# laurentsenta/testground

Hardware: AMD Instinct MI355X
Metric: simulated packets/sec (whole node) at 10k & 1M peers; % of HBM roofline (higher is better)
Workload: dtype u32/u64 integer

## Files before the change

include/tgsim.h:

```cpp
#ifndef TGSIM_H
#define TGSIM_H

#include <stddef.h>
#include <stdint.h>

#ifdef __cplusplus
extern "C" {
#endif

#define TGSIM_ABI_VERSION 2u

#define TGSIM_EXTERNAL 0xFFFFFFFFu

enum tgsim_filter { TGSIM_ACCEPT = 0, TGSIM_REJECT = 1, TGSIM_DROP = 2 };

enum tgsim_policy { TGSIM_POLICY_UNSET = 0, TGSIM_ALLOW_ALL = 1, TGSIM_DENY_ALL = 2 };

enum tgsim_verdict {
    TGSIM_V_SCHEDULED = 0,
    TGSIM_V_DISCONNECTED = 1,
    TGSIM_V_NO_ROUTE = 2,
    TGSIM_V_BLACKHOLE = 3,
    TGSIM_V_PROHIBIT = 4,
    TGSIM_V_LOSS = 5,
// ... 341 lines not shown
uint64_t tgsim_bridge_now_tick(void* bridge);
int tgsim_udp_front_create(void* bridge, uint16_t port, void** out_front);
int tgsim_udp_front_port(void* front);
int tgsim_udp_front_register(void* front, uint32_t peer, uint32_t ipv4, uint16_t port);
int tgsim_udp_front_bind_peer(void* front, uint32_t peer, uint32_t ipv4, uint16_t port);
int64_t tgsim_udp_front_pump(void* front);
void tgsim_udp_front_destroy(void* front);

double tgsim_sim_kernel_ms(void* engine, uint64_t* n_launches, int reset);
double tgsim_delivery_kernel_ms(void* engine, uint64_t* n_windows, int reset);
void* tgsim_stream(void* engine);
int64_t tgsim_debug_stamps(void* engine, uint64_t* out, size_t cap);
int64_t tgsim_debug_carry_bytes(void* engine);
int64_t tgsim_debug_bucket_records(void* engine);
int64_t tgsim_debug_fused_windows(void* engine);
int64_t tgsim_debug_sparse_windows(void* engine);
int64_t tgsim_debug_exec_faults(void);

#ifdef __cplusplus
}
#endif

#endif
```

testground_amd/abi.py:

```python
from __future__ import annotations

import ctypes as C

import numpy as np

ABI_VERSION = 2
EXTERNAL = 0xFFFFFFFF

V_SCHEDULED, V_DISCONNECTED, V_NO_ROUTE, V_BLACKHOLE, V_PROHIBIT, V_LOSS, V_QUEUE_FULL, V_EXTERNAL = range(8)
V_NONE = 15
VERDICT_NAMES = ["scheduled", "disconnected", "no_route", "blackhole", "prohibit", "loss",
                 "queue_full", "external"]

FLAG_DUP = 0x1
FLAG_CORRUPT = 0x2

OPT_DISCARD_DELIVERIES = 0x2
OPT_METRICS = 0x4
OPT_K8S = 0x8
SYNC_STATES = 65536
METRICS_SRC, METRICS_DST, METRICS_HIST = 0, 1, 2
METRICS_SRC_WORDS, METRICS_DST_WORDS, METRICS_BINS = 12, 2, 64
METRICS_SRC_COLUMNS = ["offered", "offered_bytes"] + [f"verdict_{i}" for i in range(8)] + ["served", "served_bytes"]

# ... 203 lines not shown
assert C.sizeof(FlowSummary) == 120
assert C.sizeof(FlowCC) == 16 and FLOW_CC_ROW_DTYPE.itemsize == 32 and C.sizeof(FlowCCSummary) == 64
assert C.sizeof(FlowRto) == 16 and FLOW_RTO_ROW_DTYPE.itemsize == 32 and C.sizeof(FlowRtoSummary) == 64
assert C.sizeof(FlowFb) == 16 and FLOW_FB_ROW_DTYPE.itemsize == 32 and C.sizeof(FlowFbSummary) == 96
assert C.sizeof(CommInfo) == 72 and C.sizeof(Gossip) == 24 and C.sizeof(Opts) == 56 and C.sizeof(Shape) == 56 and C.sizeof(Config) == 104

EXPORTS = [
    "tgsim_create", "tgsim_destroy", "tgsim_last_error", "tgsim_abi_version", "tgsim_configure",
    "tgsim_configure_batch", "tgsim_link_generation",
    "tgsim_submit", "tgsim_gen_storm", "tgsim_step", "tgsim_step_sim", "tgsim_deliver",
    "tgsim_deliver_async", "tgsim_wait_event", "tgsim_sync", "tgsim_step_sim_launch", "tgsim_step_sim_finish",
    "tgsim_step_sim_counts", "tgsim_delivery_event", "tgsim_step_sim_launch_slotted", "tgsim_step_sim_release",
    "tgsim_deliver_slotted_async", "tgsim_step_sim_launch_slotted_n", "tgsim_deliver_slotted_n_async",
    "tgsim_sim_capacity", "tgsim_drain", "tgsim_pending_deliveries", "tgsim_verdicts", "tgsim_stats",
    "tgsim_signal", "tgsim_signal_async", "tgsim_barrier_poll", "tgsim_sync_counters", "tgsim_sim_kernel_ms", "tgsim_delivery_kernel_ms", "tgsim_stream", "tgsim_debug_stamps",
    "tgsim_debug_fused_windows", "tgsim_debug_sparse_windows", "tgsim_debug_carry_bytes", "tgsim_debug_bucket_records", "tgsim_debug_exec_faults", "tgsim_step_n",
    "tgsim_gossip_init", "tgsim_gen_gossip", "tgsim_gossip_reached", "tgsim_gossip_spread",
    "tgsim_gossip_times", "tgsim_metrics",
    "tgsim_ping_init", "tgsim_gen_ping", "tgsim_ping_report", "tgsim_ping_pairs",
    "tgsim_flow_init", "tgsim_gen_flow", "tgsim_flow_report", "tgsim_flow_rows",
    "tgsim_flow_init_cc", "tgsim_flow_cc_rows", "tgsim_flow_cc_report",
    "tgsim_flow_init_rto", "tgsim_flow_rto_rows", "tgsim_flow_rto_report",
    "tgsim_flow_init_fb", "tgsim_flow_fb_rows", "tgsim_flow_fb_report",
    "tgsim_groups_init", "tgsim_group_matrix",
    "tgsim_comm_id", "tgsim_comm_init", "tgsim_comm_step", "tgsim_comm_launch", "tgsim_comm_finish", "tgsim_comm_run", "tgsim_comm_barrier", "tgsim_comm_info",
    "tgsim_bridge_create", "tgsim_bridge_destroy", "tgsim_bridge_send", "tgsim_bridge_step",
    "tgsim_bridge_recv", "tgsim_bridge_pending", "tgsim_bridge_in_flight", "tgsim_bridge_now_tick",
    "tgsim_bridge_link_removed",
    "tgsim_udp_front_create", "tgsim_udp_front_port", "tgsim_udp_front_register", "tgsim_udp_front_bind_peer",
    "tgsim_udp_front_pump", "tgsim_udp_front_destroy",
]
# ... 37 lines not shown
    f("sync", C.c_int, vp)
    f("sim_capacity", C.c_int64, vp)
    f("drain", C.c_int64, vp, C.c_void_p, C.c_size_t)
    f("pending_deliveries", C.c_int64, vp)
    f("verdicts", C.c_int64, vp, C.c_void_p, C.c_size_t)
    f("stats", C.c_int, vp, C.POINTER(Stats))
    f("signal", C.c_int64, vp, C.c_uint32, C.c_uint32)
    f("barrier_poll", C.c_int, vp, C.c_uint32, C.c_uint64)
    f("signal_async", C.c_int, vp, C.c_uint32, C.c_uint32)
    f("sync_counters", C.c_int, vp, C.POINTER(vp), C.POINTER(C.c_uint32), vp)
    f("sim_kernel_ms", C.c_double, vp, C.POINTER(C.c_uint64), C.c_int)
    f("delivery_kernel_ms", C.c_double, vp, C.POINTER(C.c_uint64), C.c_int)
    f("stream", vp, vp)
    f("debug_stamps", C.c_int64, vp, C.c_void_p, C.c_size_t)
    f("debug_fused_windows", C.c_int64, vp)
    f("debug_sparse_windows", C.c_int64, vp)
    f("debug_exec_faults", C.c_int64)
    f("debug_carry_bytes", C.c_int64, vp)
    f("debug_bucket_records", C.c_int64, vp)
    f("abi_version", C.c_uint32)
    f("gossip_init", C.c_int, vp, C.POINTER(Gossip))
    f("gen_gossip", C.c_int, vp, C.c_uint32)
    f("gossip_reached", C.c_int64, vp, C.c_void_p, C.c_size_t)
    f("gossip_spread", C.c_int64, vp, C.c_uint32, C.c_uint32, C.c_void_p, C.c_void_p, C.c_size_t)
    f("gossip_times", C.c_int64, vp, C.c_uint32, C.c_uint32, C.c_void_p, C.c_size_t)
    f("ping_init", C.c_int, vp, C.POINTER(Ping), C.c_void_p)
    f("gen_ping", C.c_int, vp, C.c_uint32)
    f("ping_report", C.c_int64, vp, C.POINTER(PingSummary), C.c_void_p, C.c_size_t)
    f("ping_pairs", C.c_int64, vp, C.c_uint32, C.c_uint32, C.c_void_p, C.c_size_t)
    f("flow_init", C.c_int, vp, C.POINTER(Flow), C.c_void_p, C.c_uint64)
# ... 26 lines not shown
```

testground_amd/csrc/tgsim_comm.cpp:

```cpp
#include <dlfcn.h>
#include <sched.h>
#include <errno.h>
#include <stdarg.h>
#include <stdio.h>
#include <stdlib.h>
#include <string.h>

#include <algorithm>
#include <chrono>
#include <string>
#include <vector>

#include <rccl/rccl.h>

#include "tgsim_launch.h"

using namespace tgsim;

namespace {

constexpr size_t kRec = sizeof(tgsim_delivery);
constexpr uint32_t kRoutedGridPct = 90;

struct Rccl {
// ... 453 lines not shown
  CRC(tgsim_deliver_async(e, C->in[i].p, roff[nr], C->ev_out[j]));
  CRC(tgsim_delivery_event(e, C->ev_in[i]));
  C->in_busy[i] = true;
  return 0;
}

int tgsim_comm_step(void* e, uint32_t n_ticks) {
  int rc = tgsim_comm_launch(e, n_ticks);
  return rc ? rc : tgsim_comm_finish(e);
}

int tgsim_comm_run(void* e, uint32_t n_ticks, uint32_t n_steps, uint32_t fuse, uint64_t slot_cap) {
  Comm* C = comm_of(e);
  if (!C) return e ? engine_fail(e, -EINVAL, "comm_run: no communicator (tgsim_comm_init)") : -EINVAL;
  if (C->timed_out) return -ETIMEDOUT;
  if (n_ticks == 0 || fuse == 0 || fuse > kFuseMax) return -EINVAL;
  if (C->launched) return engine_fail(e, -EBUSY, "comm_run: a launched window is not finished (tgsim_comm_finish)");
  if (engine_ping_armed(e)) return engine_fail(e, -EBUSY, "comm_run: the ping driver is armed (single engine, tgsim_step)");
  if (engine_flow_armed(e)) return engine_fail(e, -EBUSY, "comm_run: the flow driver is armed (single engine, tgsim_step)");
  if (!n_steps) return 0;
  CHIP(hipSetDevice(C->dev));
  const int nr = C->nranks;
  if (C->local) {
    CRC(tgsim_step_n(e, n_ticks, n_steps));
    C->k += n_steps;
    return 0;
  }
  if (!slot_cap) {
    uint64_t mx = 0;
    if (nr == 1) CRC(engine_route_max(e, &C->max_count));
    C->h_cnt[0] = C->max_count;
// ... 95 lines not shown
```

testground_amd/csrc/tgsim_engine.cpp:

```cpp
#include <errno.h>
#include <stdlib.h>
#include <stdarg.h>
#include <stdio.h>
#include <string.h>

#include <algorithm>
#include <array>
#include <cmath>
#include <map>
#include <numeric>
#include <string>
#include <thread>
#include <unordered_map>
#include <vector>

#include "tgsim_launch.h"

using namespace tgsim;

inline void spin_pause() {
#if defined(__x86_64__) || defined(__i386__)
  __builtin_ia32_pause();
#endif
}
// ... 322 lines not shown
  bool stamps_on = false;
  DevBuf<uint32_t> d_order;
  DevBuf<uint32_t> d_work;
  int sparse_mode = -1;
  bool rotated = false;
  bool sparse_seen = false;
  uint32_t dense_streak = 0;
  static constexpr uint32_t dense_div = 4;
  bool order_valid = false;
  struct LocalSet {
    DevBuf<tgsim_delivery> emit;
    DevBuf<uint32_t> emit_n;
  };
  LocalSet fset[2][kFuseMax];
  DevBuf<uint64_t> f_lcnt[2];
  hipEvent_t ev_fgrp[2] = {};
  uint32_t fgrp = 0;
  DevBuf<uint8_t> f_verdict[kFuseMax];
  DevBuf<uint32_t> d_done, d_ticket;
  uint32_t step_no = 0, ticket_no = 0;
  uint64_t fused_windows = 0;
  uint64_t sparse_windows = 0;
  uint32_t fused_wgs = 0;
  uint32_t routed_pct = 0;
  CommSlot comm{};
  static constexpr uint32_t prio_heavy = 512;
  int fuse_max = 8;
  DevBuf<uint64_t> d_stamps;
  uint64_t n_stamp_wg = 0;

  bool metrics_on = false;
  DevBuf<unsigned long long> d_msrc, d_mdst, d_mhist;

  bool gossip_on = false;
  bool gossip_late = false;
  tgsim_gossip gossip{};
  DevBuf<uint32_t> d_gfirst, d_gerr, d_gnbr;
  DevBuf<uint64_t> d_gfwd, d_gpend;
  DevBuf<uint64_t> d_gspread;
  DevBuf<uint32_t> d_gtimes;

  bool ping_on = false;
// ... 1241 lines not shown
  if (rc) return rc;
  HIPCHK(hipEventRecord(E->ev_dst, sq));
  rotate_emit(E);
  return 0;
}

bool fusable(Eng* E, uint32_t n_ticks, uint32_t g, bool routed = false) {
  if (g < 2 || (E->S != E->N && !routed) || !E->staged.empty() || E->gen_q.size() < g || E->metrics_on ||
      E->gossip_on || E->ping_on || E->flow_on || E->groups_on || E->sparse_mode == 1 || kSpw != 1)
    return false;
  for (uint32_t i = 0; i < g; ++i)
    if (E->gen_q[i].ticks != n_ticks || E->gen_q[i].n < 64ull * E->S) return false;
  return true;
}

struct GroupRoute {
  uint32_t n_ranks;
  const uint32_t* bounds;
  tgsim_delivery* out;
  uint64_t slot_cap;
  hipEvent_t routed;
};

int step_fused(Eng* E, uint32_t n_ticks, uint32_t g, const GroupRoute* gr = nullptr) {
  int rc = check_sim_error(E);
  if (rc) return rc;
  rc = harvest_timing(E, false);
  if (rc) return rc;
  rc = flush_config(E);
  if (rc) return rc;
// ... 9 lines not shown
    E->rotated = false;
  }
  if (E->d_done.cap < E->S) {
    HIPCHK(E->d_done.ensure(E->S));
    HIPCHK(hipMemsetAsync(E->d_done.p, 0, sizeof(uint32_t) * E->d_done.cap, E->st));
    HIPCHK(E->d_ticket.ensure(1));
    HIPCHK(hipMemsetAsync(E->d_ticket.p, 0, sizeof(uint32_t), E->st));
    E->step_no = E->ticket_no = 0;
  }
  ensure_wheel(E);
  SimArgs a = base_sim_args(E);
  const bool ordered = E->S <= kOrderMaxSources;
  a.order = ordered && E->order_valid ? E->d_order.p : nullptr;
  FusedArgs f{};
  const uint64_t nseg = static_cast<uint64_t>(g) * E->N;
  for (auto& lc : E->f_lcnt)
    if (lc.cap < static_cast<uint64_t>(kFuseMax) * E->N) {
      HIPCHK(lc.ensure(static_cast<uint64_t>(kFuseMax) * E->N));
      HIPCHK(hipMemsetAsync(lc.p, 0, sizeof(uint64_t) * lc.cap, E->st));
    }
  uint64_t rec_bound = 0, n_max = 0;
  for (uint32_t i = 0; i < g; ++i) {
    rec_bound += 2 * win[i].n + static_cast<uint64_t>(kHeapCap) * E->S;
    n_max = std::max(n_max, win[i].n);
  }
  const uint32_t n_sets = std::max(static_cast<uint32_t>(E->fuse_max), g);
  for (auto& grp : E->fset)
    for (uint32_t i = 0; i < n_sets; ++i) {
      HIPCHK(grp[i].emit.ensure(2 * n_max + static_cast<uint64_t>(kHeapCap) * E->S));
      HIPCHK(grp[i].emit_n.ensure(E->S));
    }
  HIPCHK(E->d_verdict.ensure(n_max ? n_max : 1));
  for (uint32_t i = 0; i + 1 < n_sets; ++i) HIPCHK(E->f_verdict[i].ensure(n_max ? n_max : 1));
  if (!gr) {
    const uint64_t segs = static_cast<uint64_t>(E->fuse_max) * E->N;
    const uint64_t recs = static_cast<uint64_t>(E->fuse_max) * (2 * n_max + static_cast<uint64_t>(kHeapCap) * E->S);
    HIPCHK(E->d_doff.ensure(segs + 1));
    HIPCHK(E->d_dpos.ensure(segs));
    HIPCHK(E->d_dblk.ensure((segs + 1023) / 1024 + 1));
    HIPCHK(E->d_scatter.ensure(recs));
    if (E->o.flags & TGSIM_OPT_DISCARD_DELIVERIES) HIPCHK(E->d_sorted.ensure(recs));
  }
  for (uint32_t i = 0; i < g; ++i) {
    Eng::LocalSet& ls = E->fset[p][i];
    DevBuf<uint8_t>& vb = i + 1 == g ? E->d_verdict : E->f_verdict[i];
    const uint64_t t0 = (E->now_tick + static_cast<uint64_t>(i) * n_ticks) * E->o.tick_ns;
    f.w[i] = {win[i].off.p, win[i].in.p, vb.p, ls.emit.p, ls.emit_n.p,
              gr ? nullptr : reinterpret_cast<unsigned long long*>(E->f_lcnt[p].p + static_cast<uint64_t>(i) * E->N),
              t0, t0 + n_ticks * E->o.tick_ns + E->o.lookahead_ns};
  }
  a.stamps = nullptr;
  if (E->stamps_on) {
    HIPCHK(E->d_stamps.ensure(static_cast<size_t>(g) * E->S * kStampSlots));
    a.stamps = E->d_stamps.p;
    E->n_stamp_wg = static_cast<uint64_t>(g) * E->S;
  }
  f.n_win = g;
  f.prio_n = a.order ? E->prio_heavy : 0;
  f.step_base = E->step_no;
  f.ticket_base = E->ticket_no;
  f.ticket = E->d_ticket.p;
  f.done = E->d_done.p;
  hipEvent_t ev0, ev1;
  HIPCHK(take_event(E, &ev0));
  HIPCHK(take_event(E, &ev1));
  HIPCHK(hipEventRecord(ev0, E->st));
  if (!E->fused_wgs) {
    E->fused_wgs = sim_fused_resident();
  }
  f.persistent = gr ? (E->routed_pct ? 1u : 0u) : 1u;
  const uint32_t wgs = gr && E->routed_pct ? std::max(1u, E->fused_wgs * std::min(E->routed_pct, 100u) / 100u)
                                           : E->fused_wgs;
  launch_sim_fused(a, f, wgs, E->st);
  HIPCHK(hipGetLastError());
  E->sim_calls++;
  HIPCHK(hipEventRecord(ev1, E->st));
  E->ev_pending.push_back({ev0, ev1, g});
  E->step_no += g;
  const uint32_t tickets = g * E->S;
  E->ticket_no += tickets + (f.persistent ? std::min(wgs, tickets) : 0u);
  E->fused_windows += g;
  if (ordered) {
    HIPCHK(E->d_order.ensure(E->S));
    launch_order(E->fset[p][g - 1].emit_n.p, E->S, E->d_order.p, E->st);
    HIPCHK(hipGetLastError());
    E->order_valid = true;
  }
  if (gr) {
    hipStream_t rs = E->rt_st;
    HIPCHK(hipEventRecord(E->ev_sim, E->st));
    HIPCHK(hipStreamWaitEvent(rs, E->ev_sim, 0));
    const uint64_t m = static_cast<uint64_t>(gr->n_ranks) * E->S;
    HIPCHK(E->d_rcnt.ensure(m));
    HIPCHK(E->d_rpos.ensure(m + 1));
    HIPCHK(E->d_rblk.ensure((m + 1023) / 1024 + 1));
    HIPCHK(E->d_rtot.ensure(1));
// ... 235 lines not shown
        return bail(rc);
      }
  }
  if (const char* ec = getenv("TGSIM_EMIT_COMPACT")) E->emit_compact = std::min(std::max(atoi(ec), 0), 2);
  if (const char* ds = getenv("TGSIM_DST_SLOT")) E->dst_slot = atoi(ds) != 0;
  if (const char* db = getenv("TGSIM_DST_BKT")) E->dst_bkt = atoi(db) != 0;
  E->emit_sets = E->S == E->N ? 3u : 2u;
  if (const char* es = getenv("TGSIM_EMIT_SETS")) E->emit_sets = atoi(es) == 2 ? 2u : 3u;
  if (const char* er = getenv("TGSIM_EMIT_R")) E->emit_r = static_cast<uint32_t>(std::min(std::max(1, atoi(er)), 1024));
  if (const char* ep = getenv("TGSIM_EMIT_POOL")) E->emit_pool = static_cast<uint32_t>(std::min(std::max(0, atoi(ep)), 4096));
  if (const char* ds = getenv("TGSIM_DELIVER_SLACK")) {
    E->deliver_slack = strtoull(ds, nullptr, 10);
    E->slack_forced = true;
  }
  if (const char* fz = getenv("TGSIM_FUSE")) E->fuse_max = std::max(1, std::min(atoi(fz), static_cast<int>(kFuseMax)));
  for (hipEvent_t& ev : E->ev_fgrp) {
    if ((rc = E->hip(hipEventCreateWithFlags(&ev, kEvSync), "event"))) return bail(rc);
    if ((rc = E->hip(hipEventRecord(ev, E->dst_st), "event"))) return bail(rc);
  }
  E->enabled.assign(E->N, 1);
  E->ip6_set.assign(E->N, 0);
  E->ip6.resize(E->N);
  E->k8s_init.assign(E->N, 0);
  E->gone.assign(E->N, 0);
  E->link_gen.assign(E->N, 0);
  E->ip.resize(E->N);
  for (uint32_t i = 0; i < E->N; ++i) E->ip[i] = E->o.subnet_base + 2 + i;
  E->src.resize(E->S);
  for (uint32_t s = 0; s < E->S; ++s) reset_source(E, s);
  E->patch_n = 0;
// ... 78 lines not shown
  E->d_drain.release(); E->d_gfirst.release(); E->d_gfwd.release(); E->d_gpend.release(); E->d_gnbr.release(); E->d_gerr.release(); E->d_gspread.release(); E->d_gtimes.release(); E->d_stats.release(); E->d_stamps.release(); E->d_order.release();
  E->d_msrc.release(); E->d_mdst.release(); E->d_mhist.release(); E->d_work.release(); E->d_rsend.release();
  for (auto* q : {&E->gen_q, &E->gen_free})
    for (auto& w : *q) {
      w.off.release();
      w.in.release();
    }
  for (auto* pend : {&E->ev_pending, &E->dv_pending})
    for (auto& pr : *pend) {
      (void)hipEventDestroy(pr.first);
      (void)hipEventDestroy(pr.second);
    }
  for (auto& grp : E->fset)
    for (auto& ls : grp) { ls.emit.release(); ls.emit_n.release(); }
  for (auto& v : E->f_lcnt) v.release();
  for (auto& v : E->f_verdict) v.release();
  E->d_done.release(); E->d_ticket.release();
  for (hipEvent_t ev : E->ev_fgrp)
    if (ev) (void)hipEventDestroy(ev);
  for (hipEvent_t ev : E->ev_pool) (void)hipEventDestroy(ev);
  if (E->h_err) (void)hipHostFree(E->h_err);
  if (E->h_xerr) (void)hipHostFree(E->h_xerr);
  if (E->h_work) (void)hipHostFree(E->h_work);
  flow_release(E);
  groups_release(E);
  if (E->h_ppub) (void)hipHostFree(E->h_ppub);
  if (E->ev_ping) (void)hipEventDestroy(E->ev_ping);
  if (E->ev_flow) (void)hipEventDestroy(E->ev_flow);
  if (E->ev_fb) (void)hipEventDestroy(E->ev_fb);
  if (E->h_gerr) (void)hipHostFree(E->h_gerr);
// ... 1014 lines not shown
  if (!E || n_ticks == 0 || n_ranks == 0 || n_ranks > 8 || !bounds || !d_out || slot_cap == 0) return -EINVAL;
  if (bounds[0] != 0 || bounds[n_ranks] != E->N) return E->fail(-EINVAL, "rank bounds must cover [0, n_peers)");
  if (E->route_n == Eng::kRouteSlots) return E->fail(-EBUSY, "two launched steps are not released yet");
  if (E->ping_on) return E->fail(-EBUSY, "%s: the ping driver is armed (tgsim_ping_init(engine, NULL, NULL) disarms it)", "step_sim_launch_slotted");
  if (E->flow_on) return E->fail(-EBUSY, "%s: the flow driver is armed (tgsim_flow_init(engine, NULL, NULL, 0) disarms it)", "step_sim_launch_slotted");
  HIPCHK(hipSetDevice(E->dev));
  int rc = run_sim(E, n_ticks);
  if (rc) return rc;
  return route_launch(E, n_ranks, bounds, static_cast<tgsim_delivery*>(d_out), n_ranks * (slot_cap + 1), slot_cap,
                      static_cast<hipEvent_t>(routed_event));
}

int tgsim_step_sim_launch_slotted_n(void* e, uint32_t n_ticks, uint32_t n_win, uint32_t n_ranks,
                                    const uint32_t* bounds, void* d_out, uint64_t slot_cap, void* routed_event) {
  Eng* E = as_eng(e);
  if (!E || n_ticks == 0 || n_win == 0 || n_win > kFuseMax || n_ranks == 0 || n_ranks > 8 || !bounds || !d_out ||
      slot_cap == 0)
    return -EINVAL;
  if (n_win == 1)
    return tgsim_step_sim_launch_slotted(e, n_ticks, n_ranks, bounds, d_out, slot_cap, routed_event);
  if (bounds[0] != 0 || bounds[n_ranks] != E->N) return E->fail(-EINVAL, "rank bounds must cover [0, n_peers)");
  if (E->route_n == Eng::kRouteSlots) return E->fail(-EBUSY, "two launched steps are not released yet");
  if (E->ping_on) return E->fail(-EBUSY, "%s: the ping driver is armed (tgsim_ping_init(engine, NULL, NULL) disarms it)", "step_sim_launch_slotted_n");
  if (E->flow_on) return E->fail(-EBUSY, "%s: the flow driver is armed (tgsim_flow_init(engine, NULL, NULL, 0) disarms it)", "step_sim_launch_slotted_n");
  HIPCHK(hipSetDevice(E->dev));
  if (!fusable(E, n_ticks, n_win, true))
    return E->fail(-EINVAL, "step_sim_launch_slotted_n: the next %u windows are not generated dense windows of %u ticks",
                   n_win, n_ticks);
  const GroupRoute gr{n_ranks, bounds, static_cast<tgsim_delivery*>(d_out), slot_cap, static_cast<hipEvent_t>(routed_event)};
  return step_fused(E, n_ticks, n_win, &gr);
}

int tgsim_deliver_slotted_n_async(void* e, const void* d_in, uint32_t n_ranks, uint32_t n_win, uint64_t slot_cap,
                                  void* wait_event) {
  Eng* E = as_eng(e);
  if (!E || !d_in || n_ranks == 0 || n_ranks > 8 || n_win == 0 || n_win > kFuseMax || slot_cap == 0) return -EINVAL;
  HIPCHK(hipSetDevice(E->dev));
  return deliver(E, static_cast<const tgsim_delivery*>(d_in), static_cast<uint64_t>(n_ranks) * n_win * (slot_cap + 1),
                 static_cast<hipEvent_t>(wait_event), false, slot_cap, n_win);
}

int tgsim_step_sim_release(void* e) {
  Eng* E = as_eng(e);
  if (!E) return -EINVAL;
  if (!E->route_n) return E->fail(-EINVAL, "no routed step pending");
  HIPCHK(hipSetDevice(E->dev));
  E->route_head = (E->route_head + 1) % Eng::kRouteSlots;
  E->route_n--;
  int rc = harvest_timing(E, false);
  if (rc) return rc;
  return check_sim_error(E);
// ... 76 lines not shown
  HIPCHK(E->d_bucket.ensure(cap));
  const uint32_t bounds[2] = {0, E->N};
  uint64_t count = 0;
  rc = route(E, 1, bounds, E->d_bucket.p, E->d_bucket.cap, &count);
  if (rc) return rc;
  rc = deliver(E, E->d_bucket.p, count, nullptr, true);
  if (rc) return rc;
  return finish_sim_timing(E);
}

int tgsim_step_n(void* e, uint32_t n_ticks, uint32_t n_steps) {
  Eng* E = as_eng(e);
  if (!E || n_ticks == 0) return -EINVAL;
  if (E->route_n) return E->fail(-EBUSY, "launched steps are not finished yet");
  HIPCHK(hipSetDevice(E->dev));
  while (n_steps) {
    const uint32_t g = std::min(n_steps, static_cast<uint32_t>(E->fuse_max));
    int rc;
    if (fusable(E, n_ticks, g)) {
      rc = step_fused(E, n_ticks, g);
      n_steps -= g;
    } else {
      rc = tgsim_step(e, n_ticks);
      n_steps -= 1;
    }
    if (rc) return rc;
  }
  return 0;
}

int64_t tgsim_link_generation(void* e, uint32_t peer) {
  Eng* E = as_eng(e);
  if (!E || peer >= E->N) return -EINVAL;
// ... 195 lines not shown
  return static_cast<int64_t>(n);
}

int64_t tgsim_debug_exec_faults(void) { return exec_faults(); }

int64_t tgsim_debug_sparse_windows(void* e) {
  Eng* E = as_eng(e);
  return E ? static_cast<int64_t>(E->sparse_windows) : -EINVAL;
}

int64_t tgsim_debug_fused_windows(void* e) {
  Eng* E = as_eng(e);
  return E ? static_cast<int64_t>(E->fused_windows) : -EINVAL;
}

void* tgsim_stream(void* e) {
  Eng* E = as_eng(e);
  return E ? static_cast<void*>(E->st) : nullptr;
}

int tgsim_host_compile_shape(const tgsim_shape* s, uint64_t out[13]) {
  if (!s || !out) return -EINVAL;
  const Compiled c = compile_shape(*s);
  out[0] = c.p.lat_ns; out[1] = static_cast<uint64_t>(static_cast<int64_t>(c.p.sigma));
  out[2] = static_cast<uint32_t>((s->bandwidth_bps ? s->bandwidth_bps : UINT64_MAX) / 8);
  out[3] = c.p.mult; out[4] = c.p.shift_ext & 0xFF; out[5] = c.p.burst_ns;
  out[6] = c.p.thr_loss; out[7] = c.p.thr_dup; out[8] = c.thr_cor_new; out[9] = c.p.thr_reo;
  out[10] = c.rho_dup_new; out[11] = c.rho_cor_new; out[12] = c.rho_reo_new;
  return 0;
}
// ... 19 lines not shown
```

testground_amd/csrc/tgsim_internal.h:

```cpp
#pragma once
#include <hip/hip_runtime.h>
#include <stdint.h>

#include "../../include/tgsim.h"

namespace tgsim {

constexpr uint32_t kHeapCap = 1024;
constexpr uint32_t kWave = 64;
#ifndef TGSIM_SPW
#define TGSIM_SPW 1
#endif
constexpr uint32_t kSpw = TGSIM_SPW;
constexpr uint32_t kAhead = kWave / kSpw;
constexpr uint64_t kEMask = (1ull << 46) - 1;
constexpr uint32_t kStates = TGSIM_SYNC_STATES;
constexpr uint32_t kDeadDst = 0xFFFFFFFFu;

struct alignas(16) SrcParams {
  uint64_t lat_ns;
  uint64_t burst_ns;
  int32_t sigma;
  uint32_t mult;
  uint32_t shift_ext;
// ... 101 lines not shown
  uint32_t* emit_pool_idx;
  uint32_t* g_first;
  uint64_t* g_pend;
  const uint64_t* g_fwd;
  uint32_t g_floods, g_degree;
  tgsim_delivery* dst_bkt;
  uint32_t emit_r : 24, bkt_log : 7, dst_slot : 1;
  uint32_t emit_pool_cap;
  uint4* wheel;
  WheelMeta* wmeta;
};
static_assert(sizeof(SimArgs) == 280, "SimArgs layout");
constexpr uint32_t kProfSlots = 32;
constexpr uint32_t kStampSlots = 8 + kProfSlots;

constexpr uint32_t kFuseMax = 8;
struct FusedWindow {
  const uint64_t* off;
  const InRec* in;
  uint8_t* verdict;
  tgsim_delivery* emit;
  uint32_t* emit_n;
  unsigned long long* dst_cnt;
  uint64_t t0_ns, horizon_ns;
};
struct FusedArgs {
  FusedWindow w[kFuseMax];
  uint32_t n_win;
  uint32_t step_base;
  uint32_t ticket_base;
  uint32_t* ticket;
  uint32_t* done;
  uint32_t prio_n;
  uint32_t persistent;
};
constexpr uint32_t kErrHandoff = 2u;
constexpr uint32_t kErrDeliverCap = 4u;
constexpr uint32_t kErrEmitPool = 8u;

struct EmitRead {
  const tgsim_delivery* base;
  const tgsim_delivery* pool;
  const uint32_t* pool_idx;
  uint32_t r;
  uint32_t slot;
  const tgsim_delivery* bkt;
  uint32_t bkt_log, _pad;
  const uint64_t* guard_total;
  uint64_t guard_cap;
// ... 149 lines not shown
```

testground_amd/csrc/tgsim_kernels.hip:

```cpp
#include <errno.h>
#include <stdlib.h>
#include "tgsim_fastmod.h"
#include "tgsim_launch.h"

namespace tgsim {

__device__ __forceinline__ void philox(uint32_t c0, uint32_t c1, uint32_t c2, uint32_t c3,
                                       uint32_t k0, uint32_t k1, uint32_t r[4]) {
  __asm__ volatile("" : "+s"(k0), "+s"(k1));
#pragma unroll
  for (int i = 0; i < 10; ++i) {
    const uint64_t p0 = (uint64_t)0xD2511F53u * c0, p1 = (uint64_t)0xCD9E8D57u * c2;
    const uint32_t h0 = (uint32_t)(p0 >> 32), l0 = (uint32_t)p0;
    const uint32_t h1 = (uint32_t)(p1 >> 32), l1 = (uint32_t)p1;
    const uint32_t n0 = h1 ^ c1 ^ k0, n2 = h0 ^ c3 ^ k1;
    c0 = n0; c1 = l1; c2 = n2; c3 = l0;
    k0 += 0x9E3779B9u;
    k1 += 0xBB67AE85u;
  }
  r[0] = c0; r[1] = c1; r[2] = c2; r[3] = c3;
}

__device__ __forceinline__ uint32_t crand(uint32_t raw, uint32_t rho, uint32_t& last) {
  if (rho == 0) return raw;
// ... 1513 lines not shown

__global__ __launch_bounds__(kWave, 3) void k_sim(SimArgs a) {
  __shared__ SimLdsT<kHeapCap> lds;
  const uint32_t s = a.order ? a.order[blockIdx.x] : blockIdx.x;
  if (s >= a.n_src) return;
  sim_source<false, kHeapCap>(a, s, blockIdx.x, lds);
}

__global__ __launch_bounds__(kWave, 3) void k_sim_recv(SimArgs a) {
  __shared__ SimLdsT<kHeapCap> lds;
  const uint32_t s = a.order ? a.order[blockIdx.x] : blockIdx.x;
  if (s >= a.n_src) return;
  sim_source<false, kHeapCap, kModePlain, true>(a, s, blockIdx.x, lds);
}

struct FusedSim {
  SimArgs w[kFuseMax];
};
__device__ __forceinline__ const SimArgs& kernarg_window(uint32_t k) {
  using KernargSimArgs = __attribute__((address_space(4))) const SimArgs;
  const KernargSimArgs* ka =
      (KernargSimArgs*)((__attribute__((address_space(4))) const char*)__builtin_amdgcn_kernarg_segment_ptr() +
                        k * sizeof(SimArgs));
  return *(const SimArgs*)ka;
}

__global__ __launch_bounds__(kWave, 3) void k_sim_fused(FusedSim fs, FusedArgs f) {
  const SimArgs& a0 = fs.w[0];
  __shared__ SimLdsT<kHeapCap> lds;
  const uint32_t total = f.n_win * a0.n_src;
  uint32_t t = 0;
  if (threadIdx.x == 0) t = atomicAdd(f.ticket, 1u) - f.ticket_base;
  t = (uint32_t)__builtin_amdgcn_readfirstlane((int)t);
  while (t < total) {
    const uint32_t k = t / a0.n_src, pos = t - k * a0.n_src;
    const uint32_t s = a0.order ? a0.order[pos] : pos;
    if (pos < f.prio_n) __builtin_amdgcn_s_setprio(3);
    else __builtin_amdgcn_s_setprio(0);
    if (k) {
      const uint32_t need = f.step_base + k;
      uint32_t late = 0;
      if (threadIdx.x == 0) {
// ... 9 lines not shown
      if (__builtin_amdgcn_readfirstlane((int)late) && threadIdx.x == 0) {
        atomicOr(&a0.stats[kStErr], (unsigned long long)kErrHandoff);
        if (a0.err_host)
          __hip_atomic_store(a0.err_host, (uint64_t)kErrHandoff, __ATOMIC_RELAXED, __HIP_MEMORY_SCOPE_SYSTEM);
      }
    }
    const uint32_t next = sim_source<false, kHeapCap, kModeHandoff>(kernarg_window(k), s, t, lds,
                                                            f.persistent ? f.ticket : nullptr, f.ticket_base);
    __asm__ volatile("s_waitcnt vmcnt(0)" ::: "memory");
    if (threadIdx.x == 0)
      __hip_atomic_store(f.done + s, f.step_base + k + 1, __ATOMIC_RELAXED, __HIP_MEMORY_SCOPE_AGENT);
    if (!f.persistent) break;
    t = next;
  }
}

constexpr uint32_t kSparseQ = 4;
constexpr uint32_t kFifoRounds = 4;

__device__ __forceinline__ bool emit_record(const SimArgs& a, const EmitOut& eo, bool live, const uint4& x, uint64_t d,
                                            uint32_t xlen, uint32_t src, uint32_t fw, uint32_t fw_f,
                                            uint32_t& emitted, uint64_t below) {
  unsigned long long rank = 0;
  if (live && a.dst_cnt) {
    if (a.dst_slot) rank = atomicAdd(&a.dst_cnt[x.w], 1ull);
    else atomicAdd(&a.dst_cnt[x.w], 1ull);
  }
  const bool inb = live && a.dst_bkt != nullptr && rank < (1ull << a.bkt_log);
  bool ov = live && !inb;
  const uint32_t i = emitted + (uint32_t)__popcll(__ballot(ov) & below);
// ... 2761 lines not shown

__global__ __launch_bounds__(256) void k_group_read(unsigned long long* m, unsigned long long* out, uint32_t words,
                                                    uint32_t reset) {
  const uint32_t i = blockIdx.x * 256 + threadIdx.x;
  if (i >= words) return;
  out[i] = m[i];
  if (reset) m[i] = 0ull;
}


void launch_sim(const SimArgs& a, uint32_t n_wg, hipStream_t st) {
  if (a.g_first) hipLaunchKernelGGL(k_sim_recv, dim3(n_wg), dim3(kWave), 0, st, a);
  else hipLaunchKernelGGL(k_sim, dim3(n_wg), dim3(kWave), 0, st, a);
}

void launch_sim_fused(const SimArgs& a, const FusedArgs& f, uint32_t n_wg, hipStream_t st) {
  const uint32_t total = f.n_win * a.n_src;
  FusedSim fs;
  for (uint32_t k = 0; k < kFuseMax; ++k) {
    fs.w[k] = a;
    if (k >= f.n_win) continue;
    const FusedWindow& w = f.w[k];
    fs.w[k].off = w.off;
    fs.w[k].in = w.in;
    fs.w[k].verdict = w.verdict;
    fs.w[k].emit = w.emit;
    fs.w[k].emit_n = w.emit_n;
    fs.w[k].dst_cnt = w.dst_cnt;
    fs.w[k].t0_ns = w.t0_ns;
    fs.w[k].horizon_ns = w.horizon_ns;
  }
  const dim3 grid(f.persistent && n_wg < total ? n_wg : total);
  hipLaunchKernelGGL(k_sim_fused, grid, dim3(kWave), 0, st, fs, f);
}

uint32_t sim_fused_resident() {
  int dev = 0, per_cu = 0, cus = 0;
  if (hipGetDevice(&dev) != hipSuccess ||
      hipDeviceGetAttribute(&cus, hipDeviceAttributeMultiprocessorCount, dev) != hipSuccess ||
      hipOccupancyMaxActiveBlocksPerMultiprocessor(&per_cu, k_sim_fused, kWave, 0) != hipSuccess || per_cu <= 0)
    return 2048;
  return (uint32_t)(per_cu * cus);
}

__global__ void k_work_done(SparseWork work, uint32_t* host) {
  const uint32_t i = threadIdx.x;
  if (i < 2)
    __hip_atomic_store(&host[i], *(i ? work.multi_n() : work.list_n()), __ATOMIC_RELAXED, __HIP_MEMORY_SCOPE_SYSTEM);
// ... 469 lines not shown
```

testground_amd/csrc/tgsim_launch.h:

```cpp
#pragma once
#include "tgsim_internal.h"

namespace tgsim {

struct GenArgsHost {
  uint32_t tab[16];
  uint32_t k0, k1, n_src, shard_begin, n_peers, n_ticks;
  uint64_t now_tick;
};

struct RouteArgsHost {
  EmitRead emit;
  const uint32_t* emit_n;
  const uint64_t* off;
  uint32_t n_src;
  uint32_t n_ranks;
  uint32_t bounds[9];
  uint64_t* cnt;
  const uint64_t* pos;
  tgsim_delivery* out;
  uint64_t out_cap;
  uint64_t slot_cap;
  uint64_t chunk_stride;
  uint32_t waves_per_block;
};

void launch_sim(const SimArgs& a, uint32_t n_wg, hipStream_t st);
void launch_sim_fused(const SimArgs& a, const FusedArgs& f, uint32_t n_wg, hipStream_t st);
uint32_t sim_fused_resident();
void launch_sim_sparse(const SimArgs& a, hipStream_t st, uint32_t* work_host, uint32_t list_hint);
void launch_order(const uint32_t* weight, uint32_t n, uint32_t* order, hipStream_t st);
void launch_apply_cfg(const CfgPatch* p, uint32_t n, SrcParams* params, SrcState* state,
                      unsigned long long* stats, hipStream_t st);
void launch_purge(uint4* heap, uint4* wheel, const WheelMeta* wmeta, const SrcState* state, uint32_t n_src,
                  const uint8_t* gone, hipStream_t st);
void launch_unrotate(uint4* heap, SrcState* state, uint32_t n_src, hipStream_t st);
void launch_publish(const uint64_t* v0, const uint32_t* v1, uint64_t* slot, uint64_t seq, hipStream_t st);
void launch_signal(unsigned long long* table, uint64_t* mirror, uint32_t state, uint32_t n, uint64_t* result,
                   uint64_t* marker, uint64_t seq, hipStream_t st);
void launch_gen(const GenArgsHost& h, uint64_t* counts, const uint64_t* off, uint32_t* gen_seq,
                InRec* out, int phase, hipStream_t st);
void launch_gossip(const GossipArgs& g, const tgsim_delivery* recs, uint64_t n, uint64_t* counts,
                   const uint64_t* off, InRec* out, int phase, hipStream_t st, uint64_t out_cap = 0,
// ... 70 lines not shown
```

Baseline: 39.07 billion.

## Fuse up to 32 windows per launch via device-side window descriptors

Raises the maximum number of simulation windows fused into one persistent kernel launch from 8 to 32. For groups larger than 8, a small kernel writes per-window SimArgs descriptors to device memory, which the fused kernel reads through the constant address space, because kernarg space cannot hold 32 full copies. Group sizes are balanced across the step count, with a tail heuristic and a memory-budget cap that shrinks the fuse width when the per-window buffers would exceed free HBM. This is meant to cut launch and window-boundary overhead, at the cost of more device memory, an extra descriptor kernel launch, and longer cross-window handoff chains.

```diff
diff --git a/include/tgsim.h b/include/tgsim.h
--- a/include/tgsim.h
+++ b/include/tgsim.h
@@ -379,6 +379,7 @@
 int64_t tgsim_debug_carry_bytes(void* engine);
 int64_t tgsim_debug_bucket_records(void* engine);
 int64_t tgsim_debug_fused_windows(void* engine);
+int64_t tgsim_debug_fused_launches(void* engine);
 int64_t tgsim_debug_sparse_windows(void* engine);
 int64_t tgsim_debug_exec_faults(void);
 
diff --git a/testground_amd/abi.py b/testground_amd/abi.py
--- a/testground_amd/abi.py
+++ b/testground_amd/abi.py
@@ -241,7 +241,7 @@
     "tgsim_deliver_slotted_async", "tgsim_step_sim_launch_slotted_n", "tgsim_deliver_slotted_n_async",
     "tgsim_sim_capacity", "tgsim_drain", "tgsim_pending_deliveries", "tgsim_verdicts", "tgsim_stats",
     "tgsim_signal", "tgsim_signal_async", "tgsim_barrier_poll", "tgsim_sync_counters", "tgsim_sim_kernel_ms", "tgsim_delivery_kernel_ms", "tgsim_stream", "tgsim_debug_stamps",
-    "tgsim_debug_fused_windows", "tgsim_debug_sparse_windows", "tgsim_debug_carry_bytes", "tgsim_debug_bucket_records", "tgsim_debug_exec_faults", "tgsim_step_n",
+    "tgsim_debug_fused_windows", "tgsim_debug_fused_launches", "tgsim_debug_sparse_windows", "tgsim_debug_carry_bytes", "tgsim_debug_bucket_records", "tgsim_debug_exec_faults", "tgsim_step_n",
     "tgsim_gossip_init", "tgsim_gen_gossip", "tgsim_gossip_reached", "tgsim_gossip_spread",
     "tgsim_gossip_times", "tgsim_metrics",
     "tgsim_ping_init", "tgsim_gen_ping", "tgsim_ping_report", "tgsim_ping_pairs",
@@ -309,6 +309,7 @@
     f("stream", vp, vp)
     f("debug_stamps", C.c_int64, vp, C.c_void_p, C.c_size_t)
     f("debug_fused_windows", C.c_int64, vp)
+    f("debug_fused_launches", C.c_int64, vp)
     f("debug_sparse_windows", C.c_int64, vp)
     f("debug_exec_faults", C.c_int64)
     f("debug_carry_bytes", C.c_int64, vp)
diff --git a/testground_amd/csrc/tgsim_comm.cpp b/testground_amd/csrc/tgsim_comm.cpp
--- a/testground_amd/csrc/tgsim_comm.cpp
+++ b/testground_amd/csrc/tgsim_comm.cpp
@@ -491,7 +491,7 @@
   Comm* C = comm_of(e);
   if (!C) return e ? engine_fail(e, -EINVAL, "comm_run: no communicator (tgsim_comm_init)") : -EINVAL;
   if (C->timed_out) return -ETIMEDOUT;
-  if (n_ticks == 0 || fuse == 0 || fuse > kFuseMax) return -EINVAL;
+  if (n_ticks == 0 || fuse == 0 || fuse > kFuseMaxSharded) return -EINVAL;
   if (C->launched) return engine_fail(e, -EBUSY, "comm_run: a launched window is not finished (tgsim_comm_finish)");
   if (engine_ping_armed(e)) return engine_fail(e, -EBUSY, "comm_run: the ping driver is armed (single engine, tgsim_step)");
   if (engine_flow_armed(e)) return engine_fail(e, -EBUSY, "comm_run: the flow driver is armed (single engine, tgsim_step)");
diff --git a/testground_amd/csrc/tgsim_engine.cpp b/testground_amd/csrc/tgsim_engine.cpp
--- a/testground_amd/csrc/tgsim_engine.cpp
+++ b/testground_amd/csrc/tgsim_engine.cpp
@@ -360,18 +360,24 @@
   };
   LocalSet fset[2][kFuseMax];
   DevBuf<uint64_t> f_lcnt[2];
+  DevBuf<SimArgs> f_desc;
+  uint32_t fuse_sets = 0;
+  uint32_t fuse_cap = 0;
+  uint64_t fuse_set_recs = 0;
+  uint64_t fuse_held = 0;
+  int64_t fuse_mem_mb = -1;
   hipEvent_t ev_fgrp[2] = {};
   uint32_t fgrp = 0;
   DevBuf<uint8_t> f_verdict[kFuseMax];
   DevBuf<uint32_t> d_done, d_ticket;
   uint32_t step_no = 0, ticket_no = 0;
-  uint64_t fused_windows = 0;
+  uint64_t fused_windows = 0, fused_launches = 0;
   uint64_t sparse_windows = 0;
   uint32_t fused_wgs = 0;
   uint32_t routed_pct = 0;
   CommSlot comm{};
   static constexpr uint32_t prio_heavy = 512;
-  int fuse_max = 8;
+  int fuse_max = 32;
   DevBuf<uint64_t> d_stamps;
   uint64_t n_stamp_wg = 0;
 
@@ -1643,6 +1649,71 @@
   return true;
 }
 
+constexpr uint32_t kFuseFloor = 8;
+constexpr uint32_t kFuseTail = 6, kTailWinUs = 25, kBoundaryUs = 180;
+uint32_t fuse_tail(uint32_t n, uint32_t cap) {
+  if (cap < kFuseFloor || n <= kFuseTail) return 0;
+  const uint32_t k_plain = (n + cap - 1) / cap, last_plain = n / k_plain;
+  const uint32_t k_tail = (n - kFuseTail + cap - 1) / cap + 1;
+  if (last_plain <= kFuseTail) return 0;
+  return kTailWinUs * (last_plain - kFuseTail) > kBoundaryUs * (k_tail - k_plain) ? kFuseTail : 0;
+}
+uint32_t fuse_next_group(uint32_t n, uint32_t cap, uint32_t tail) {
+  if (cap < kFuseFloor) return std::min(n, cap);
+  const uint32_t body = n > tail ? n - tail : n;
+  const uint32_t k = (body + cap - 1) / cap;
+  return (body + k - 1) / k;
+}
+uint32_t fuse_largest_group(uint32_t n, uint32_t cap) { return n ? fuse_next_group(n, cap, fuse_tail(n, cap)) : 0; }
+
+int fuse_group_cap(Eng* E, uint32_t n_ticks, uint32_t n_steps, uint32_t* cap_out) {
+  const uint32_t want = static_cast<uint32_t>(E->fuse_max), floor = std::min(want, kFuseFloor);
+  *cap_out = E->fuse_cap ? std::min(E->fuse_cap, want) : want;
+  if (n_steps < 2 || E->S != E->N) return 0;
+  uint64_t n_max = 0;
+  for (size_t i = 0; i < E->gen_q.size(); ++i)
+    if (E->gen_q[i].ticks == n_ticks) n_max = std::max(n_max, E->gen_q[i].n);
+  if (n_max < 64ull * E->S) return 0;
+  const uint64_t set_recs = 2 * n_max + static_cast<uint64_t>(kHeapCap) * E->S;
+  const uint32_t ahead = E->gen_q.size() > n_steps ? static_cast<uint32_t>(std::min<size_t>(E->gen_q.size() - n_steps, 1u << 20)) : 0;
+  const auto sets_at = [&](uint32_t cap) {
+    return std::max(fuse_largest_group(n_steps, cap), fuse_largest_group(ahead, cap));
+  };
+  uint32_t cap = *cap_out, sets = sets_at(cap);
+  if (sets <= E->fuse_sets && set_recs <= E->fuse_set_recs) return 0;
+  if (sets > floor) {
+    const auto grown = [](uint64_t n) { return n + n / 2; };
+    const uint64_t copies = (E->o.flags & TGSIM_OPT_DISCARD_DELIVERIES) ? 4 : 3;
+    const uint64_t per_win = copies * grown(set_recs) * sizeof(tgsim_delivery) + grown(n_max) +
+                             2 * grown(E->S) * sizeof(uint32_t) + 4ull * E->N * sizeof(uint64_t);
+    uint64_t budget;
+    if (E->fuse_mem_mb >= 0) {
+      budget = static_cast<uint64_t>(E->fuse_mem_mb) << 20;
+    } else {
+      size_t free_b = 0, total_b = 0;
+      HIPCHK(hipMemGetInfo(&free_b, &total_b));
+      budget = (free_b + E->fuse_held) / 2;
+    }
+    if (sets * per_win > budget) {
+      cap = static_cast<uint32_t>(std::min<uint64_t>(cap, std::max<uint64_t>(floor, budget / per_win)));
+      sets = sets_at(cap);
+      E->fuse_cap = cap;
+      for (auto& grp : E->fset)
+        for (uint32_t i = sets; i < kFuseMax; ++i) {
+          grp[i].emit.release();
+          grp[i].emit_n.release();
+        }
+      for (uint32_t i = sets; i < kFuseMax; ++i) E->f_verdict[i].release();
+      E->fuse_sets = std::min(E->fuse_sets, sets);
+    }
+    E->fuse_held = std::max(sets, E->fuse_sets) * per_win;
+  }
+  E->fuse_set_recs = std::max(E->fuse_set_recs, set_recs);
+  E->fuse_sets = std::max(E->fuse_sets, sets);
+  *cap_out = cap;
+  return 0;
+}
+
 struct GroupRoute {
   uint32_t n_ranks;
   const uint32_t* bounds;
@@ -1682,17 +1753,19 @@
   a.order = ordered && E->order_valid ? E->d_order.p : nullptr;
   FusedArgs f{};
   const uint64_t nseg = static_cast<uint64_t>(g) * E->N;
+  const uint32_t n_sets = std::max({E->fuse_sets, g, gr ? std::min(static_cast<uint32_t>(E->fuse_max), kFuseMaxSharded) : 0u});
+  E->fuse_sets = n_sets;
   for (auto& lc : E->f_lcnt)
-    if (lc.cap < static_cast<uint64_t>(kFuseMax) * E->N) {
-      HIPCHK(lc.ensure(static_cast<uint64_t>(kFuseMax) * E->N));
+    if (lc.cap < static_cast<uint64_t>(n_sets) * E->N) {
+      HIPCHK(lc.ensure_exact(static_cast<uint64_t>(n_sets) * E->N));
       HIPCHK(hipMemsetAsync(lc.p, 0, sizeof(uint64_t) * lc.cap, E->st));
     }
+  if (g > kFuseMaxSharded) HIPCHK(E->f_desc.ensure_exact(kFuseMax));
   uint64_t rec_bound = 0, n_max = 0;
   for (uint32_t i = 0; i < g; ++i) {
     rec_bound += 2 * win[i].n + static_cast<uint64_t>(kHeapCap) * E->S;
     n_max = std::max(n_max, win[i].n);
   }
-  const uint32_t n_sets = std::max(static_cast<uint32_t>(E->fuse_max), g);
   for (auto& grp : E->fset)
     for (uint32_t i = 0; i < n_sets; ++i) {
       HIPCHK(grp[i].emit.ensure(2 * n_max + static_cast<uint64_t>(kHeapCap) * E->S));
@@ -1701,8 +1774,8 @@
   HIPCHK(E->d_verdict.ensure(n_max ? n_max : 1));
   for (uint32_t i = 0; i + 1 < n_sets; ++i) HIPCHK(E->f_verdict[i].ensure(n_max ? n_max : 1));
   if (!gr) {
-    const uint64_t segs = static_cast<uint64_t>(E->fuse_max) * E->N;
-    const uint64_t recs = static_cast<uint64_t>(E->fuse_max) * (2 * n_max + static_cast<uint64_t>(kHeapCap) * E->S);
+    const uint64_t segs = static_cast<uint64_t>(n_sets) * E->N;
+    const uint64_t recs = static_cast<uint64_t>(n_sets) * (2 * n_max + static_cast<uint64_t>(kHeapCap) * E->S);
     HIPCHK(E->d_doff.ensure(segs + 1));
     HIPCHK(E->d_dpos.ensure(segs));
     HIPCHK(E->d_dblk.ensure((segs + 1023) / 1024 + 1));
@@ -1729,6 +1802,7 @@
   f.ticket_base = E->ticket_no;
   f.ticket = E->d_ticket.p;
   f.done = E->d_done.p;
+  f.desc = E->f_desc.p;
   hipEvent_t ev0, ev1;
   HIPCHK(take_event(E, &ev0));
   HIPCHK(take_event(E, &ev1));
@@ -1739,7 +1813,7 @@
   f.persistent = gr ? (E->routed_pct ? 1u : 0u) : 1u;
   const uint32_t wgs = gr && E->routed_pct ? std::max(1u, E->fused_wgs * std::min(E->routed_pct, 100u) / 100u)
                                            : E->fused_wgs;
-  launch_sim_fused(a, f, wgs, E->st);
+  if (launch_sim_fused(a, f, wgs, E->st)) return E->fail(-EINVAL, "step_fused: a group of %u windows cannot be launched", g);
   HIPCHK(hipGetLastError());
   E->sim_calls++;
   HIPCHK(hipEventRecord(ev1, E->st));
@@ -1748,6 +1822,7 @@
   const uint32_t tickets = g * E->S;
   E->ticket_no += tickets + (f.persistent ? std::min(wgs, tickets) : 0u);
   E->fused_windows += g;
+  E->fused_launches++;
   if (ordered) {
     HIPCHK(E->d_order.ensure(E->S));
     launch_order(E->fset[p][g - 1].emit_n.p, E->S, E->d_order.p, E->st);
@@ -2013,6 +2088,7 @@
     E->slack_forced = true;
   }
   if (const char* fz = getenv("TGSIM_FUSE")) E->fuse_max = std::max(1, std::min(atoi(fz), static_cast<int>(kFuseMax)));
+  if (const char* fm = getenv("TGSIM_FUSE_MEM_MB")) E->fuse_mem_mb = std::max(0ll, atoll(fm));
   for (hipEvent_t& ev : E->ev_fgrp) {
     if ((rc = E->hip(hipEventCreateWithFlags(&ev, kEvSync), "event"))) return bail(rc);
     if ((rc = E->hip(hipEventRecord(ev, E->dst_st), "event"))) return bail(rc);
@@ -2121,6 +2197,7 @@
   for (auto& grp : E->fset)
     for (auto& ls : grp) { ls.emit.release(); ls.emit_n.release(); }
   for (auto& v : E->f_lcnt) v.release();
+  E->f_desc.release();
   for (auto& v : E->f_verdict) v.release();
   E->d_done.release(); E->d_ticket.release();
   for (hipEvent_t ev : E->ev_fgrp)
@@ -3165,7 +3242,7 @@
 int tgsim_step_sim_launch_slotted_n(void* e, uint32_t n_ticks, uint32_t n_win, uint32_t n_ranks,
                                     const uint32_t* bounds, void* d_out, uint64_t slot_cap, void* routed_event) {
   Eng* E = as_eng(e);
-  if (!E || n_ticks == 0 || n_win == 0 || n_win > kFuseMax || n_ranks == 0 || n_ranks > 8 || !bounds || !d_out ||
+  if (!E || n_ticks == 0 || n_win == 0 || n_win > kFuseMaxSharded || n_ranks == 0 || n_ranks > 8 || !bounds || !d_out ||
       slot_cap == 0)
     return -EINVAL;
   if (n_win == 1)
@@ -3185,7 +3262,7 @@
 int tgsim_deliver_slotted_n_async(void* e, const void* d_in, uint32_t n_ranks, uint32_t n_win, uint64_t slot_cap,
                                   void* wait_event) {
   Eng* E = as_eng(e);
-  if (!E || !d_in || n_ranks == 0 || n_ranks > 8 || n_win == 0 || n_win > kFuseMax || slot_cap == 0) return -EINVAL;
+  if (!E || !d_in || n_ranks == 0 || n_ranks > 8 || n_win == 0 || n_win > kFuseMaxSharded || slot_cap == 0) return -EINVAL;
   HIPCHK(hipSetDevice(E->dev));
   return deliver(E, static_cast<const tgsim_delivery*>(d_in), static_cast<uint64_t>(n_ranks) * n_win * (slot_cap + 1),
                  static_cast<hipEvent_t>(wait_event), false, slot_cap, n_win);
@@ -3292,9 +3369,12 @@
   if (!E || n_ticks == 0) return -EINVAL;
   if (E->route_n) return E->fail(-EBUSY, "launched steps are not finished yet");
   HIPCHK(hipSetDevice(E->dev));
+  uint32_t cap = 1;
+  int rc = fuse_group_cap(E, n_ticks, n_steps, &cap);
+  if (rc) return rc;
+  const uint32_t tail = fuse_tail(n_steps, cap);
   while (n_steps) {
-    const uint32_t g = std::min(n_steps, static_cast<uint32_t>(E->fuse_max));
-    int rc;
+    const uint32_t g = fuse_next_group(n_steps, cap, tail);
     if (fusable(E, n_ticks, g)) {
       rc = step_fused(E, n_ticks, g);
       n_steps -= g;
@@ -3520,6 +3600,11 @@
   return E ? static_cast<int64_t>(E->fused_windows) : -EINVAL;
 }
 
+int64_t tgsim_debug_fused_launches(void* e) {
+  Eng* E = as_eng(e);
+  return E ? static_cast<int64_t>(E->fused_launches) : -EINVAL;
+}
+
 void* tgsim_stream(void* e) {
   Eng* E = as_eng(e);
   return E ? static_cast<void*>(E->st) : nullptr;
diff --git a/testground_amd/csrc/tgsim_internal.h b/testground_amd/csrc/tgsim_internal.h
--- a/testground_amd/csrc/tgsim_internal.h
+++ b/testground_amd/csrc/tgsim_internal.h
@@ -139,7 +139,8 @@
 constexpr uint32_t kProfSlots = 32;
 constexpr uint32_t kStampSlots = 8 + kProfSlots;
 
-constexpr uint32_t kFuseMax = 8;
+constexpr uint32_t kFuseMax = 32;
+constexpr uint32_t kFuseMaxSharded = 8;
 struct FusedWindow {
   const uint64_t* off;
   const InRec* in;
@@ -158,6 +159,22 @@
   uint32_t* done;
   uint32_t prio_n;
   uint32_t persistent;
+  SimArgs* desc;
+};
+struct FusedArgs8 {
+  FusedWindow w[kFuseMaxSharded];
+  uint32_t n_win, step_base, ticket_base;
+  uint32_t* ticket;
+  uint32_t* done;
+  uint32_t prio_n, persistent;
+};
+struct FusedCtl {
+  uint32_t n_win, step_base, ticket_base, prio_n, persistent, n_src;
+  uint32_t* ticket;
+  uint32_t* done;
+  const uint32_t* order;
+  unsigned long long* stats;
+  uint64_t* err_host;
 };
 constexpr uint32_t kErrHandoff = 2u;
 constexpr uint32_t kErrDeliverCap = 4u;
diff --git a/testground_amd/csrc/tgsim_kernels.hip b/testground_amd/csrc/tgsim_kernels.hip
--- a/testground_amd/csrc/tgsim_kernels.hip
+++ b/testground_amd/csrc/tgsim_kernels.hip
@@ -1551,8 +1551,67 @@
   sim_source<false, kHeapCap, kModePlain, true>(a, s, blockIdx.x, lds);
 }
 
+__device__ __forceinline__ const SimArgs& desc_window(const SimArgs* desc, uint32_t k) {
+  using ConstSimArgs = __attribute__((address_space(4))) const SimArgs;
+  return *(const SimArgs*)((ConstSimArgs*)desc + k);
+}
+__global__ __launch_bounds__(kWave) void k_fused_desc(SimArgs a, FusedArgs f) {
+  const uint32_t k = blockIdx.x;
+  if (k >= f.n_win || threadIdx.x) return;
+  const FusedWindow& w = f.w[k];
+  a.off = w.off;
+  a.in = w.in;
+  a.verdict = w.verdict;
+  a.emit = w.emit;
+  a.emit_n = w.emit_n;
+  a.dst_cnt = w.dst_cnt;
+  a.t0_ns = w.t0_ns;
+  a.horizon_ns = w.horizon_ns;
+  f.desc[k] = a;
+}
+
+__global__ __launch_bounds__(kWave, 3) void k_sim_fused(const SimArgs* desc, FusedCtl f) {
+  __shared__ SimLdsT<kHeapCap> lds;
+  const uint32_t total = f.n_win * f.n_src;
+  uint32_t t = 0;
+  if (threadIdx.x == 0) t = atomicAdd(f.ticket, 1u) - f.ticket_base;
+  t = (uint32_t)__builtin_amdgcn_readfirstlane((int)t);
+  while (t < total) {
+    const uint32_t k = t / f.n_src, pos = t - k * f.n_src;
+    const uint32_t s = f.order ? f.order[pos] : pos;
+    if (pos < f.prio_n) __builtin_amdgcn_s_setprio(3);
+    else __builtin_amdgcn_s_setprio(0);
+    if (k) {
+      const uint32_t need = f.step_base + k;
+      uint32_t late = 0;
+      if (threadIdx.x == 0) {
+        for (uint32_t spin = 0;
+             (int32_t)(__hip_atomic_load(f.done + s, __ATOMIC_RELAXED, __HIP_MEMORY_SCOPE_AGENT) - need) < 0;) {
+          __builtin_amdgcn_s_sleep(2);
+          if (++spin > (1u << 22)) {
+            late = 1;
+            break;
+          }
+        }
+      }
+      if (__builtin_amdgcn_readfirstlane((int)late) && threadIdx.x == 0) {
+        atomicOr(&f.stats[kStErr], (unsigned long long)kErrHandoff);
+        if (f.err_host)
+          __hip_atomic_store(f.err_host, (uint64_t)kErrHandoff, __ATOMIC_RELAXED, __HIP_MEMORY_SCOPE_SYSTEM);
+      }
+    }
+    const uint32_t next = sim_source<false, kHeapCap, kModeHandoff>(desc_window(desc, k), s, t, lds,
+                                                            f.persistent ? f.ticket : nullptr, f.ticket_base);
+    __asm__ volatile("s_waitcnt vmcnt(0)" ::: "memory");
+    if (threadIdx.x == 0)
+      __hip_atomic_store(f.done + s, f.step_base + k + 1, __ATOMIC_RELAXED, __HIP_MEMORY_SCOPE_AGENT);
+    if (!f.persistent) break;
+    t = next;
+  }
+}
+
 struct FusedSim {
-  SimArgs w[kFuseMax];
+  SimArgs w[kFuseMaxSharded];
 };
 __device__ __forceinline__ const SimArgs& kernarg_window(uint32_t k) {
   using KernargSimArgs = __attribute__((address_space(4))) const SimArgs;
@@ -1562,7 +1621,7 @@
   return *(const SimArgs*)ka;
 }
 
-__global__ __launch_bounds__(kWave, 3) void k_sim_fused(FusedSim fs, FusedArgs f) {
+__global__ __launch_bounds__(kWave, 3) void k_sim_fused8(FusedSim fs, FusedArgs8 f) {
   const SimArgs& a0 = fs.w[0];
   __shared__ SimLdsT<kHeapCap> lds;
   const uint32_t total = f.n_win * a0.n_src;
@@ -1602,6 +1661,7 @@
     t = next;
   }
 }
+
 
 constexpr uint32_t kSparseQ = 4;
 constexpr uint32_t kFifoRounds = 4;
@@ -4393,24 +4453,42 @@
   else hipLaunchKernelGGL(k_sim, dim3(n_wg), dim3(kWave), 0, st, a);
 }
 
-void launch_sim_fused(const SimArgs& a, const FusedArgs& f, uint32_t n_wg, hipStream_t st) {
+int launch_sim_fused(const SimArgs& a, const FusedArgs& f, uint32_t n_wg, hipStream_t st) {
   const uint32_t total = f.n_win * a.n_src;
-  FusedSim fs;
-  for (uint32_t k = 0; k < kFuseMax; ++k) {
-    fs.w[k] = a;
-    if (k >= f.n_win) continue;
-    const FusedWindow& w = f.w[k];
-    fs.w[k].off = w.off;
-    fs.w[k].in = w.in;
-    fs.w[k].verdict = w.verdict;
-    fs.w[k].emit = w.emit;
-    fs.w[k].emit_n = w.emit_n;
-    fs.w[k].dst_cnt = w.dst_cnt;
-    fs.w[k].t0_ns = w.t0_ns;
-    fs.w[k].horizon_ns = w.horizon_ns;
-  }
+  if (!total || f.n_win > kFuseMax) return -EINVAL;
   const dim3 grid(f.persistent && n_wg < total ? n_wg : total);
-  hipLaunchKernelGGL(k_sim_fused, grid, dim3(kWave), 0, st, fs, f);
+  if (f.n_win <= kFuseMaxSharded) {
+    FusedSim fs;
+    FusedArgs8 f8{};
+    for (uint32_t k = 0; k < kFuseMaxSharded; ++k) {
+      fs.w[k] = a;
+      if (k >= f.n_win) continue;
+      const FusedWindow& w = f8.w[k] = f.w[k];
+      fs.w[k].off = w.off;
+      fs.w[k].in = w.in;
+      fs.w[k].verdict = w.verdict;
+      fs.w[k].emit = w.emit;
+      fs.w[k].emit_n = w.emit_n;
+      fs.w[k].dst_cnt = w.dst_cnt;
+      fs.w[k].t0_ns = w.t0_ns;
+      fs.w[k].horizon_ns = w.horizon_ns;
+    }
+    f8.n_win = f.n_win;
+    f8.step_base = f.step_base;
+    f8.ticket_base = f.ticket_base;
+    f8.ticket = f.ticket;
+    f8.done = f.done;
+    f8.prio_n = f.prio_n;
+    f8.persistent = f.persistent;
+    hipLaunchKernelGGL(k_sim_fused8, grid, dim3(kWave), 0, st, fs, f8);
+    return 0;
+  }
+  if (!f.desc) return -EINVAL;
+  hipLaunchKernelGGL(k_fused_desc, dim3(f.n_win), dim3(kWave), 0, st, a, f);
+  const FusedCtl c{f.n_win, f.step_base, f.ticket_base, f.prio_n, f.persistent, a.n_src,
+                   f.ticket,  f.done,    a.order,       a.stats,  a.err_host};
+  hipLaunchKernelGGL(k_sim_fused, grid, dim3(kWave), 0, st, (const SimArgs*)f.desc, c);
+  return 0;
 }
 
 uint32_t sim_fused_resident() {
diff --git a/testground_amd/csrc/tgsim_launch.h b/testground_amd/csrc/tgsim_launch.h
--- a/testground_amd/csrc/tgsim_launch.h
+++ b/testground_amd/csrc/tgsim_launch.h
@@ -26,7 +26,7 @@
 };
 
 void launch_sim(const SimArgs& a, uint32_t n_wg, hipStream_t st);
-void launch_sim_fused(const SimArgs& a, const FusedArgs& f, uint32_t n_wg, hipStream_t st);
+int launch_sim_fused(const SimArgs& a, const FusedArgs& f, uint32_t n_wg, hipStream_t st);
 uint32_t sim_fused_resident();
 void launch_sim_sparse(const SimArgs& a, hipStream_t st, uint32_t* work_host, uint32_t list_hint);
 void launch_order(const uint32_t* weight, uint32_t n, uint32_t* order, hipStream_t st);
```

After: 40.83 billion (median of 6 runs). 1.05x the previous value.
